# juliohm/GeoStatsSolvers.jl

Hardware: AMD Instinct MI355X
Metric: kriged domain points/sec (OK, 1000 3-D data, Matern-3/2, global neighbourhood) (higher is better)
Workload: dtype f64; 1 GPU; configs[1]: OK, 1000 3-D data -> 1000000 domain points per GPU, Matern-3/2 range 30, global neighbourhood; step = device fit + predict; points_per_gpu=1000000, ndata=1000, factor=replicated

## Files before the change

geostatssolvers.jl_amd/csrc/cokrig.hip:

```cpp
#include "krig_handle.h"
#include "mfma_f64.h"

#include <cmath>
#include <cstring>
#include <vector>

namespace gss {

template <int DIM>
__global__ __launch_bounds__(256) void cokrig_system_kernel(VgDev vg, const double* __restrict__ xd,
                                                            const int* __restrict__ var,
                                                            const double* __restrict__ tab, int n,
                                                            double* __restrict__ M, int64_t ldw) {
  const int j = blockIdx.x * 256 + threadIdx.x;
  const int i0 = blockIdx.y * 64;
  const int i1 = i0 + 64 < n ? i0 + 64 : n;
  if (j >= n) return;
  double c[DIM];
#pragma unroll
  for (int k = 0; k < DIM; ++k) c[k] = xd[(int64_t)j * DIM + k];
  const int vj = var[j];
  for (int i = i0; i < i1; ++i) {
    double x[DIM];
#pragma unroll
// ... 263 lines not shown
  for (int a = 0; a < nz; ++a) {
    h->c00[a] = tab[CO_C0 + a * CO_MAXZ + a];
    h->means[a] = tab[CO_MEANS + a];
  }
  std::memset(&h->ds, 0, sizeof(h->ds));
  h->ds.variant = variant;
  h->ds.dim = dim;
  for (int k = 0; k < 3; ++k) h->ds.inv_scale[k] = 1.0;
  h->nc = variant == GSS_KRIG_ORDINARY ? nz : 0;
  h->ds.nc = h->nc;
  h->N1 = n + h->nc;
  h->N1pad = round_up(h->N1 + 1, BK);
  h->ldw = round_up(h->N1 + 1, BM);

  hipStream_t s = to_stream(stream);
  GSS_TRY(h->z.alloc(sizeof(double) * (size_t)n));
  GSS_TRY(h->covar.alloc(sizeof(int32_t) * (size_t)n));
  GSS_TRY(h->cotab.alloc(sizeof(tab)));
  GSS_TRY(krig_upload_samples(h->fr, xdata, n, dim, &h->xdata, &h->xraw, s));
  GSS_HIP(hipMemcpyAsync(h->z.p, z, sizeof(double) * n, hipMemcpyHostToDevice, s));
  GSS_HIP(hipMemcpyAsync(h->covar.p, var, sizeof(int32_t) * n, hipMemcpyHostToDevice, s));
  GSS_HIP(hipMemcpyAsync(h->cotab.p, tab, sizeof(tab), hipMemcpyHostToDevice, s));
  {
    std::vector<double> xg((size_t)(n * dim)), zr((size_t)n);
    std::vector<int32_t> row((size_t)n);
    int64_t at[CO_MAXZ];
    h->co_off[0] = 0;
    for (int a = 0; a < CO_MAXZ; ++a) {
      at[a] = h->co_off[a];
      h->co_off[a + 1] = h->co_off[a] + per[a];
    }
    for (int64_t i = 0; i < n; ++i) {
      const int64_t j = at[var[i]]++;
      for (int k = 0; k < dim; ++k) xg[(size_t)(j * dim + k)] = xdata[i * dim + k];
      zr[(size_t)j] = z[i] - tab[CO_MEANS + var[i]];
      row[(size_t)j] = (int32_t)i;
    }
    GSS_TRY(h->co_zres.alloc(sizeof(double) * (size_t)n));
    GSS_TRY(h->co_row.alloc(sizeof(int32_t) * (size_t)n));
    GSS_TRY(krig_upload_samples(h->fr, xg.data(), n, dim, &h->co_xg, &h->co_xg_raw, s));
    GSS_HIP(hipMemcpyAsync(h->co_zres.p, zr.data(), sizeof(double) * n, hipMemcpyHostToDevice, s));
    GSS_HIP(hipMemcpyAsync(h->co_row.p, row.data(), sizeof(int32_t) * n, hipMemcpyHostToDevice, s));
    GSS_HIP(hipStreamSynchronize(s));
  }
  if (factor) {
    const bool async = (flags & GSS_KRIG_ASYNC_FIT) != 0;
    GSS_TRY(krig_factorize(h, s, async));
    if (!async) GSS_TRY(krig_fit_wait(h));
  }
  guard.h = nullptr;
  *out = h;
  return GSS_OK;
}

extern "C" {

int32_t gss_cokrig_create(gss_krig_t** out, const gss_variogram_t* structure, int32_t nz, const double* b0,
                          const double* b1, int32_t variant, const double* means, const double* xdata,
                          const double* z, const int32_t* var, int64_t n, int32_t flags, void* stream) {
  GSS_ENTRY();
  return cokrig_create_impl("gss_cokrig_create", true, out, structure, nz, b0, b1, variant, means, xdata, z, var, n,
                            flags, stream);
}

int32_t gss_cokrig_create_local(gss_krig_t** out, const gss_variogram_t* structure, int32_t nz, const double* b0,
                                const double* b1, int32_t variant, const double* means, const double* xdata,
                                const double* z, const int32_t* var, int64_t n, void* stream) {
  GSS_ENTRY();
  return cokrig_create_impl("gss_cokrig_create_local", false, out, structure, nz, b0, b1, variant, means, xdata, z, var,
                            n, 0, stream);
}

int32_t gss_cokrig_predict_global(gss_krig_t* h, const double* xdom, int64_t m, double* mean, double* variance,
                                  uint8_t* status, int32_t mem, void* stream) {
  GSS_ENTRY();
  GSS_REQUIRE(h != nullptr, "NULL handle");
  GSS_REQUIRE(h->nz > 0, "gss_cokrig_predict_global: the handle is not a cokriging system (gss_cokrig_create makes one)");
  GSS_REQUIRE(h->factored, "handle has no factor");
  GSS_REQUIRE(m >= 0 && (m == 0 || (xdom && mean && variance)), "gss_cokrig_predict_global: NULL array");
  if (m == 0) return GSS_OK;
  hipStream_t s = to_stream(stream);
  const int dim = h->dim, nz = h->nz;
  GSS_TRY(krig_quadform_attrs());

  int64_t mc = cokrig_chunk_cap(krig_chunk_points(h->N1pad * nz, m));
  DomainCall dc;
  Staged& sx = *dc.in(xdom, sizeof(double) * dim);
  Staged& smean = *dc.out(mean, sizeof(double), nz);
  Staged& svar = *dc.out(variance, sizeof(double), nz);
  Staged& sstat = *dc.out(status, 1, nz);
  GSS_TRY(dc.begin(mem, m, s, true, &h->fr));
  if (dc.piped && mc > HostPipe::PIECE) mc = HostPipe::PIECE;
  double *Rws = nullptr, *mpart = nullptr;
  GSS_TRY(krig_workspace(h->N1pad * nz, mc, s, &Rws, &mpart));
  const int64_t ldr = mc, blk = h->N1pad * ldr;
  const int seg_len = (int)((h->n + NSEG - 1) / NSEG);

  for (int64_t off = 0; off < m; off += mc) {
    const int64_t mv = (m - off) < mc ? (m - off) : mc;
    const int64_t cols = round_up(mv, 256);
    const double* x0 = sx.as<double>() + off * dim;
    GSS_TRY(dc.pipe.fetch(off, mv, s));
    const int nblk = (int)(cols / 256);
    const int nrows = (int)(h->N1pad - h->n);
    {
      ProfScope ps("cokrig_rhs", s);
      const double* xd = h->xdata.as<double>();
      const int* cv = h->covar.as<int>();
      const double* tab = h->cotab.as<double>();
      switch (dim) {
        case 1: GSS_TRY(launch_cokrig_rhs<1>(s, h->vg, xd, cv, tab, nz, (int)h->n, x0, mv, Rws, ldr, blk, seg_len, nblk)); break;
        case 2: GSS_TRY(launch_cokrig_rhs<2>(s, h->vg, xd, cv, tab, nz, (int)h->n, x0, mv, Rws, ldr, blk, seg_len, nblk)); break;
        default: GSS_TRY(launch_cokrig_rhs<3>(s, h->vg, xd, cv, tab, nz, (int)h->n, x0, mv, Rws, ldr, blk, seg_len, nblk)); break;
      }
      hipLaunchKernelGGL(cokrig_tail_rows_kernel, dim3((unsigned)(cols / 256)), dim3(256), 0, s, Rws, ldr, blk,
                         (int)h->n, h->nc, nrows, nz, cols);
      GSS_HIP(hipGetLastError());
    }
    GSS_TRY(krig_join_device(h, s));
    {
      ProfScope pq("krig_quadform", s);
      for (int t = 0; t < nz; ++t) {
        uint8_t* stp = status ? sstat.as<uint8_t>() + t * m + off : nullptr;
        launch_krig_quadform(h, Rws + t * blk, ldr, h->c00[t], h->means[t], mv, cols,
                             smean.as<double>() + t * m + off, svar.as<double>() + t * m + off, stp, mpart, s);
      }
    }
    GSS_HIP(hipGetLastError());
    GSS_TRY(dc.pipe.deliver(off, mv, s));
  }
  GSS_TRY(dc.finish(s));
  return krig_fit_wait(h);
}

int32_t gss_cokrig_predict_knn(gss_krig_t* h, const double* xdom, int64_t m, const int32_t* k, int32_t minneighbors,
                               double radius, const double* inv_radii, int32_t metric, double metric_param,
                               double* mean, double* variance, uint8_t* status, int32_t* idx_out, int32_t* count_out,
                               int32_t mem, void* stream) {
  GSS_ENTRY();
  GSS_REQUIRE(h != nullptr, "NULL handle");
  GSS_REQUIRE(h->nz > 0, "gss_cokrig_predict_knn: the handle is not a cokriging system (gss_cokrig_create and "
              "gss_cokrig_create_local make one)");
  const int nz = h->nz, dim = h->dim;
  int ksum = 0;
  GSS_TRY(cokrig_knn_counts(h, "gss_cokrig_predict_knn", "; gss_cokrig_predict_global uses every sample", k, &ksum));
  GSS_REQUIRE(m >= 0 && (m == 0 || (xdom && mean && variance)), "gss_cokrig_predict_knn: NULL array");

  hipStream_t s = to_stream(stream);
  CoGrouped g;
  cokrig_grouped(h, &g);
  Searcher sr[COL_MAXZ];
  GSS_TRY(cokrig_searchers(h, g, sr, metric, metric_param, radius, inv_radii, s));
  if (m == 0) return GSS_OK;
  DomainCall dc;
  dc.in(xdom, sizeof(double) * dim);
  Staged& smean = *dc.out(mean, sizeof(double), nz);
  Staged& svar = *dc.out(variance, sizeof(double), nz);
  Staged& sstat = *dc.out(status, 1, nz);
  Staged& sidx = *dc.out(idx_out, sizeof(int32_t) * (size_t)ksum);
  Staged& scnt = *dc.out(count_out, sizeof(int32_t) * (size_t)nz);
  GSS_TRY(dc.begin(mem, m, s, !sr[0].two_frames, &h->fr));
  GSS_TRY(cokrig_local_dev(h->vg, h->variant, dim, g, sr, k, minneighbors, dc.x(), sr[0].two_frames ? dc.x_raw : nullptr,
                           m, smean.as<double>(), svar.as<double>(), sstat.as<uint8_t>(), m, sidx.as<int>(),
                           scnt.as<int>(), s, &dc.pipe));
  return dc.finish(s);
}
// ... 3 lines not shown
```

geostatssolvers.jl_amd/csrc/krig.hip:

```cpp
#include "krig_handle.h"

#include "mfma_f64.h"

#include <mutex>

#include <cmath>
#include <cstdlib>
#include <cstring>
#include <type_traits>
#include <vector>

namespace gss {

template <int DIM>
__global__ __launch_bounds__(256) void drift_rows_kernel(DriftSpec ds, const double* __restrict__ x,
                                                         const double* __restrict__ drift_vals, int64_t npts,
                                                         int64_t ncols_pad, double* __restrict__ out, int64_t ld,
                                                         int nrows) {
  const int64_t p = (int64_t)blockIdx.x * 256 + threadIdx.x;
  if (p >= ncols_pad) return;
  const int64_t pc = p < npts ? p : npts - 1;
  double xs[DIM];
#pragma unroll
  for (int k = 0; k < DIM; ++k) xs[k] = (x[pc * DIM + k] - ds.center[k]) * ds.inv_scale[k];
// ... 468 lines not shown
    if (v > 0) ws = (size_t)v << 20;
  }
  int64_t cap = (int64_t)(ws / (sizeof(double) * (size_t)N1pad));
  const int64_t round = 512 * 128;
  cap = cap >= round ? cap / round * round : cap / 256 * 256;
  if (cap < 256) cap = 256;
  return round_up(m, 256) < cap ? round_up(m, 256) : cap;
}

struct KrigWorkspace {
  DevBuf R, mean_part;
  int64_t doubles = 0, mc = 0, nI = 0;
};
static KrigWorkspace g_ws;

int32_t gss::krig_workspace(int64_t N1pad, int64_t mc, hipStream_t s, double** R, double** mean_part) {
  const int64_t nI = (N1pad + BM - 1) / BM + 1;
  if (g_ws.doubles < N1pad * mc || g_ws.mc < mc || g_ws.nI < nI) {
    GSS_HIP(hipStreamSynchronize(s));
    g_ws.R.release();
    g_ws.mean_part.release();
    GSS_TRY(g_ws.R.alloc(sizeof(double) * (size_t)(N1pad * mc)));
    GSS_TRY(g_ws.mean_part.alloc(sizeof(double) * (size_t)((NSEG + 1 + nI) * mc)));
    g_ws.doubles = N1pad * mc;
    g_ws.mc = mc;
    g_ws.nI = nI;
  }
  *R = g_ws.R.as<double>();
  *mean_part = g_ws.mean_part.as<double>();
  return GSS_OK;
}

static int32_t launch_drift_rows(const gss_krig* h, const double* x, const double* drift_vals, int64_t npts,
                                 int64_t ncols_pad, double* out, int64_t ld, int nrows, hipStream_t s) {
  dim3 grid((unsigned)((ncols_pad + 255) / 256));
  switch (h->dim) {
    case 1:
      hipLaunchKernelGGL((drift_rows_kernel<1>), grid, dim3(256), 0, s, h->ds, x, drift_vals, npts, ncols_pad, out,
                         ld, nrows);
      break;
    case 2:
      hipLaunchKernelGGL((drift_rows_kernel<2>), grid, dim3(256), 0, s, h->ds, x, drift_vals, npts, ncols_pad, out,
                         ld, nrows);
      break;
    default:
      hipLaunchKernelGGL((drift_rows_kernel<3>), grid, dim3(256), 0, s, h->ds, x, drift_vals, npts, ncols_pad, out,
                         ld, nrows);
      break;
  }
  GSS_HIP(hipGetLastError());
  return GSS_OK;
}

__global__ void small_gram_kernel(const double* __restrict__ Bm, int nc, int64_t n, double* __restrict__ S, int lds) {
  const int c = blockIdx.x, c2 = blockIdx.y;
  if (c2 > c) return;
  double acc = 0.0;
  for (int64_t i = threadIdx.x; i < n; i += 64) acc = fma(Bm[(int64_t)c * n + i], Bm[(int64_t)c2 * n + i], acc);
#pragma unroll
  for (int off = 32; off >= 1; off >>= 1) acc += __shfl_xor(acc, off);
  if (threadIdx.x == 0) {
    S[c + c2 * lds] = acc;
    S[c2 + c * lds] = acc;
  }
}

__global__ void constraint_rows_kernel(const double* __restrict__ WS, int64_t ldws, const double* __restrict__ T,
                                       int nc, int64_t n, double* __restrict__ Wp_rows, int64_t ldw) {
  const int64_t j = (int64_t)blockIdx.x * 256 + threadIdx.x;
  if (j >= n) return;
  for (int i = 0; i < nc; ++i) {
    double acc = 0.0;
    for (int c = 0; c <= i; ++c) acc = fma(WS[i + c * ldws], T[(int64_t)c * n + j], acc);
    Wp_rows[i + j * ldw] = -acc;
  }
}

__global__ __launch_bounds__(256) void wd_row_kernel(const double* __restrict__ wd, int64_t N1,
                                                     double* __restrict__ row, int64_t ldw) {
  const int64_t k = (int64_t)blockIdx.x * 256 + threadIdx.x;
  if (k < N1) row[k * ldw] = wd[k];
}

struct FitPlan {
  double *M, *T, *Dinv, *Fd, *Bm, *S, *SDinv, *gwork, *zz, *u;
  int *info, *info2;
  int64_t szM, szS;
};

static int32_t krig_fit_plan(gss_krig* h, FitPlan* fp) {
  const int64_t n = h->n, N1pad = h->N1pad, ldw = h->ldw;
  const int64_t szM = ldw * N1pad;
  int64_t szT = n * n > (int64_t)MAX_NC * n ? n * n : (int64_t)MAX_NC * n;
  if (potrf_inverse_work_doubles(n) > szT) szT = potrf_inverse_work_doubles(n);
  const int64_t szDinv = 64 * 64;
  const int64_t szFd = (int64_t)MAX_NC * n, szBm = (int64_t)MAX_NC * n;
  const int64_t szS = 2 * MAX_NC * MAX_NC + 64 * 64;
  int64_t szGemv = gemv_work_doubles(false, ldw, ldw);
  if (gemv_work_doubles(true, ldw, ldw) > szGemv) szGemv = gemv_work_doubles(true, ldw, ldw);
  const int64_t szVec = 2 * ldw;
  DevBuf& ws = h->fit_ws;
  GSS_TRY(ws.alloc(sizeof(double) * (size_t)(szM + szT + szDinv + szFd + szBm + szS + szGemv + szVec) + 64));
  fp->M = ws.as<double>();
  fp->T = fp->M + szM;
  fp->Dinv = fp->T + szT;
  fp->Fd = fp->Dinv + szDinv;
  fp->Bm = fp->Fd + szFd;
  fp->S = fp->Bm + szBm;
  fp->SDinv = fp->S + MAX_NC * MAX_NC;
  fp->gwork = fp->S + szS;
  fp->zz = fp->gwork + szGemv;
  fp->u = fp->zz + ldw;
  fp->info = reinterpret_cast<int*>(fp->u + ldw);
  fp->info2 = fp->info + 1;
  fp->szM = szM;
  fp->szS = szS;
  return GSS_OK;
}

static int32_t krig_fit_enqueue(gss_krig* h, const FitPlan& fp, hipStream_t s) {
  const int64_t n = h->n, N1 = h->N1, ldw = h->ldw;
  const int nc = h->nc;
  double *M = fp.M, *T = fp.T, *Fd = fp.Fd, *Bm = fp.Bm, *S = fp.S, *SDinv = fp.SDinv;
  double *gwork = fp.gwork, *zz = fp.zz, *u = fp.u;
  int *info = fp.info, *info2 = fp.info2;
  const int64_t szM = fp.szM, szS = fp.szS;
  GSS_TRY(dev_zero_bytes(M, sizeof(double) * (size_t)szM, s));
  GSS_TRY(dev_zero_bytes(h->factor.p, h->factor.bytes, s));
  GSS_TRY(dev_zero_bytes(info2, sizeof(int), s));
  if (h->nz > 0) {
    GSS_TRY(cokrig_fit_system(h, M, s));
  } else {
    GSS_TRY(cov_pairwise_dev(h->vg, h->xdata.as<double>(), n, h->xdata.as<double>(), n, M, ldw, s));
  }
  double* Wp = h->Wp();
  GSS_TRY(potrf_inverse_f64(M, n, ldw, Wp, ldw, T, info, false, s, true));

  if (nc > 0) {
    GSS_TRY(dev_zero_bytes(S, sizeof(double) * (size_t)szS, s));
    if (h->nz > 0) {
      GSS_TRY(cokrig_fit_indicators(h, Fd, s));
    } else {
      GSS_TRY(launch_drift_rows(h, h->xdata.as<double>(), h->drift_data.as<double>(), n, n, Fd, n, nc, s));
    }
    for (int c = 0; c < nc; ++c) GSS_TRY(gemv_f64(false, n, n, Wp, ldw, Fd + (int64_t)c * n, Bm + (int64_t)c * n, gwork, s));
    hipLaunchKernelGGL(small_gram_kernel, dim3(nc, nc), dim3(64), 0, s, Bm, nc, n, S, MAX_NC);
    GSS_HIP(hipGetLastError());
    GSS_TRY(potrf_inverse_f64(S, nc, MAX_NC, Wp + n + n * ldw, ldw, SDinv, info2, false, s));
    for (int c = 0; c < nc; ++c) GSS_TRY(gemv_f64(true, n, n, Wp, ldw, Bm + (int64_t)c * n, T + (int64_t)c * n, gwork, s));
    hipLaunchKernelGGL(constraint_rows_kernel, dim3((unsigned)((n + 255) / 256)), dim3(256), 0, s, Wp + n + n * ldw, ldw, T,
                       nc, n, Wp + n, ldw);
    GSS_HIP(hipGetLastError());
  }

  GSS_TRY(dev_zero_bytes(zz, sizeof(double) * (size_t)(2 * ldw), s));
  GSS_TRY(dev_copy_f64(zz, h->z.as<double>(), n, s));
  if (h->nz > 0) {
    if (h->variant == GSS_KRIG_SIMPLE) cokrig_fit_center(h, zz, s);
  } else if (h->variant == GSS_KRIG_SIMPLE && h->sk_mean != 0.0) {
    hipLaunchKernelGGL(sub_scalar_kernel, dim3((unsigned)((n + 255) / 256)), dim3(256), 0, s, zz, n, h->sk_mean);
  }
  GSS_TRY(gemv_f64(false, N1, N1, Wp, ldw, zz, u, gwork, s));
  if (nc > 0) hipLaunchKernelGGL(flip_tail_kernel, dim3(1), dim3(256), 0, s, u, n, N1);
  GSS_TRY(gemv_f64(true, N1, N1, Wp, ldw, u, h->wd(), gwork, s));
  hipLaunchKernelGGL(wd_row_kernel, dim3((unsigned)((N1 + 255) / 256)), dim3(256), 0, s, h->wd(), N1, Wp + N1, ldw);
  GSS_HIP(hipGetLastError());
  return GSS_OK;
}

static hipStream_t krig_fit_stream() { return helper_stream(HELPER_FIT); }

static int32_t krig_factor_alloc(gss_krig* h) {
  if (h->factor.p) return GSS_OK;
  return h->factor.alloc(sizeof(double) * (size_t)(h->ldw * h->N1pad + h->N1pad));
}

int32_t gss::krig_factorize(gss_krig* h, hipStream_t s, bool async) {
  GSS_TRY(krig_factor_alloc(h));
  hipStream_t fs = s;
  if (async) {
    fs = krig_fit_stream();
    if (!fs) {
      async = false;
      fs = s;
    }
  }
  if (async) {
    ScopedEvent e0;
    GSS_HIP(e0.create());
    GSS_HIP(hipEventRecord(e0, s));
    GSS_HIP(hipStreamWaitEvent(fs, e0, 0));
    if (!h->fit_info_host) GSS_HIP(hipHostMalloc(reinterpret_cast<void**>(&h->fit_info_host), 2 * sizeof(int), hipHostMallocDefault));
  }
  FitPlan fp;
  GSS_TRY(krig_fit_plan(h, &fp));
  GSS_TRY(krig_fit_enqueue(h, fp, fs));
  h->fit_info = fp.info;
  h->fit_stream = fs;
  h->fit_async = async;
  if (async) GSS_HIP(hipMemcpyAsync(h->fit_info_host, fp.info, 2 * sizeof(int), hipMemcpyDeviceToHost, fs));
  if (!h->fit_done) GSS_HIP(hipEventCreateWithFlags(&h->fit_done, hipEventDisableTiming));
  GSS_HIP(hipEventRecord(h->fit_done, fs));
  h->fit_pending = true;
  h->factored = true;
  return GSS_OK;
}

int32_t gss::krig_join_device(gss_krig* h, hipStream_t s) {
  if (h->fit_pending && h->fit_done && h->fit_stream != s) GSS_HIP(hipStreamWaitEvent(s, h->fit_done, 0));
  return GSS_OK;
}

int32_t gss::krig_fit_wait(gss_krig* h) {
  if (!h->fit_pending) return GSS_OK;
  h->fit_pending = false;
  GSS_HIP(hipEventSynchronize(h->fit_done));
  int hinfo[2] = {0, 0};
  if (h->fit_async) {
    hinfo[0] = h->fit_info_host[0];
    hinfo[1] = h->fit_info_host[1];
  } else {
    GSS_HIP(hipMemcpy(hinfo, h->fit_info, 2 * sizeof(int), hipMemcpyDeviceToHost));
  }
  h->fit_ws.release();
  h->fit_info = nullptr;
  if (hinfo[0] < 0) {
    h->factored = false;
    static thread_local bool retrying = false;
    if (!retrying) {
      potrf_panel_disable();
      retrying = true;
      int32_t rc = krig_factorize(h, h->fit_stream, false);
      if (rc == GSS_OK) rc = krig_fit_wait(h);
      retrying = false;
      return rc;
    }
    set_error("kriging fit: the factorisation kernel gave up waiting at a grid barrier");
    return GSS_ERR_HIP;
  }
  if (hinfo[0] != 0) {
    h->factored = false;
    set_error("kriging covariance matrix is not positive definite (pivot %d of %lld); add a nugget or remove "
              "duplicate samples", hinfo[0] - 1, (long long)h->n);
    return GSS_ERR_NOT_POSDEF;
  }
  if (hinfo[1] != 0) {
    h->factored = false;
    set_error("drift functions are linearly dependent on the sample locations (constraint %d)", hinfo[1] - 1);
    return GSS_ERR_NOT_POSDEF;
  }
  return GSS_OK;
}

void gss::launch_krig_quadform(const gss_krig* h, const double* Rws, int64_t ldr, double c00, double mean0,
                                 int64_t mv, int64_t cols, double* mean_out, double* var_out, uint8_t* stp,
                                 double* qpart, hipStream_t s) {
  const int nstrips = (int)(cols / BN);
  const int nI = (int)((h->N1 + BM) / BM);
#define GSS_K3_ARGS(S0, NS) h->Wp(), h->ldw, (int)h->N1pad, (int)h->n, (int)h->N1, Rws, ldr, c00, mean0, mv, \
                            mean_out, var_out, stp, qpart, (S0), (NS)
  const int nmain = (nstrips / 512) * 512;
  const int nrem = nstrips - nmain;
  if (nmain > 0)
    hipLaunchKernelGGL((krig_quadform_kernel<false>), dim3((unsigned)nmain), dim3(256), QUADFORM_LDS_BYTES, s,
                       GSS_K3_ARGS(0, nmain));
  if (nrem > 0) {
    const unsigned grid = (unsigned)(8 * ((nrem + 7) / 8) * nI);
    hipLaunchKernelGGL((krig_quadform_kernel<true>), dim3(grid), dim3(256), QUADFORM_LDS_BYTES, s,
                       GSS_K3_ARGS(nmain, nrem));
    const int64_t pbeg = (int64_t)nmain * BN;
    if (mv > pbeg)
      hipLaunchKernelGGL(krig_finish_kernel, dim3((unsigned)((mv - pbeg + 255) / 256)), dim3(256), 0, s, qpart + pbeg,
                         nI, ldr, c00, mv - pbeg, var_out + pbeg, stp ? stp + pbeg : nullptr);
  }
#undef GSS_K3_ARGS
}

int32_t gss::krig_quadform_attrs() {
  static uint64_t attr_set = 0;
  if (first_on_this_device(attr_set)) {
    GSS_HIP(hipFuncSetAttribute(reinterpret_cast<const void*>(krig_quadform_kernel<false>),
                                hipFuncAttributeMaxDynamicSharedMemorySize, (int)QUADFORM_LDS_BYTES));
    GSS_HIP(hipFuncSetAttribute(reinterpret_cast<const void*>(krig_quadform_kernel<true>),
                                hipFuncAttributeMaxDynamicSharedMemorySize, (int)QUADFORM_LDS_BYTES));
  }
  return GSS_OK;
}

int32_t gss::krig_upload_samples(const Frame& fr, const double* xhost, int64_t n, int dim, DevBuf* x, DevBuf* xraw,
                                 hipStream_t s) {
  const size_t bytes = sizeof(double) * (size_t)(n * dim);
  GSS_TRY(x->alloc(bytes));
  if (!fr.on) {
    GSS_HIP(hipMemcpyAsync(x->p, xhost, bytes, hipMemcpyHostToDevice, s));
    return GSS_OK;
  }
  GSS_TRY(xraw->alloc(bytes));
  GSS_HIP(hipMemcpyAsync(xraw->p, xhost, bytes, hipMemcpyHostToDevice, s));
  return frame_apply_dev(fr, xraw->as<double>(), n, x->as<double>(), s);
// ... 66 lines not shown
      break;
    }
    case GSS_KRIG_EXTDRIFT:
      GSS_REQUIRE(ndrift >= 1 && ndrift <= MAX_NC && drift_data != nullptr, "external drift needs 1..%d drifts",
                  MAX_NC);
      h->nc = ndrift;
      break;
    default:
      GSS_REQUIRE(false, "unknown kriging variant %d", variant);
  }
  h->ds.nc = h->nc;
  if ((flags & GSS_KRIG_NO_FACTOR) == 0)
    GSS_REQUIRE(n + h->nc >= 1 && n >= h->nc, "fewer samples (%lld) than drift constraints (%d)", (long long)n,
                h->nc);
  h->N1 = n + h->nc;
  h->N1pad = round_up(h->N1 + 1, BK);
  h->ldw = round_up(h->N1 + 1, BM);

  hipStream_t s = to_stream(stream);
  GSS_TRY(h->z.alloc(sizeof(double) * (size_t)n));
  GSS_TRY(krig_upload_samples(h->fr, xdata, n, h->dim, &h->xdata, &h->xraw, s));
  GSS_HIP(hipMemcpyAsync(h->z.p, z, sizeof(double) * n, hipMemcpyHostToDevice, s));
  if (variant == GSS_KRIG_EXTDRIFT) {
    GSS_TRY(h->drift_data.alloc(sizeof(double) * (size_t)(n * ndrift)));
    GSS_HIP(hipMemcpyAsync(h->drift_data.p, drift_data, sizeof(double) * n * ndrift, hipMemcpyHostToDevice, s));
  }
  GSS_HIP(hipStreamSynchronize(s));
  if ((flags & GSS_KRIG_NO_FACTOR) == 0) {
    const bool async = (flags & GSS_KRIG_ASYNC_FIT) != 0;
    GSS_TRY(krig_factorize(h, s, async));
    if (!async) GSS_TRY(krig_fit_wait(h));
  }
  guard.h = nullptr;
  *out = h;
  return GSS_OK;
}

int32_t gss_krig_destroy(gss_krig_t* h) {
  GSS_ENTRY();
  delete h;
  return GSS_OK;
}

int32_t gss_krig_info(const gss_krig_t* h, int64_t* n, int32_t* nc) {
  GSS_ENTRY();
  GSS_REQUIRE(h != nullptr, "NULL handle");
  if (n) *n = h->n;
  if (nc) *nc = h->nc;
  return GSS_OK;
}

int32_t gss_krig_factor_buffer(gss_krig_t* h, void** dev_ptr, int64_t* bytes) {
  GSS_ENTRY();
  GSS_REQUIRE(h != nullptr && dev_ptr != nullptr && bytes != nullptr, "NULL argument");
  GSS_TRY(krig_fit_wait(h));
  GSS_TRY(krig_factor_alloc(h));
  *dev_ptr = h->factor.p;
  *bytes = (int64_t)(sizeof(double) * (size_t)(h->ldw * h->N1pad + h->N1pad));
  return GSS_OK;
}

int32_t gss_krig_adopt_factor(gss_krig_t* h) {
  GSS_ENTRY();
  GSS_REQUIRE(h != nullptr, "NULL handle");
  GSS_REQUIRE(h->factor.p != nullptr, "gss_krig_adopt_factor: no factor has arrived (gss_krig_factor_buffer hands out "
                                      "the buffer to fill)");
  h->factored = true;
  return GSS_OK;
}

int32_t gss_krig_predict_global(gss_krig_t* h, const double* xdom, const double* drift_dom, int64_t m,
                                double* mean, double* var, uint8_t* status, int32_t mem, void* stream) {
  GSS_ENTRY();
  GSS_REQUIRE(h != nullptr, "NULL handle");
  GSS_TRY(krig_refuse_cokrig(h, "gss_krig_predict_global"));
  GSS_REQUIRE(h->factored, "handle has no factor (created with GSS_KRIG_NO_FACTOR and never adopted one)");
  GSS_REQUIRE(m >= 0 && (m == 0 || (xdom && mean && var)), "gss_krig_predict_global: NULL array");
  GSS_REQUIRE(h->variant != GSS_KRIG_EXTDRIFT || drift_dom != nullptr, "external drift values missing");
  if (m == 0) return GSS_OK;
  hipStream_t s = to_stream(stream);
  const int dim = h->dim;

  GSS_TRY(krig_quadform_attrs());

  int64_t mc = krig_chunk_points(h->N1pad, m);
  DomainCall dc;
  Staged& sx = *dc.in(xdom, sizeof(double) * dim);
  Staged& sd = *dc.in(h->variant == GSS_KRIG_EXTDRIFT ? drift_dom : nullptr, sizeof(double) * h->ndrift);
  Staged& smean = *dc.out(mean, sizeof(double));
  Staged& svar = *dc.out(var, sizeof(double));
  Staged& sstat = *dc.out(status, 1);
  GSS_TRY(dc.begin(mem, m, s, true, &h->fr));
  if (dc.piped && mc > HostPipe::PIECE) mc = HostPipe::PIECE;
  double *Rws = nullptr, *mpart = nullptr;
  GSS_TRY(krig_workspace(h->N1pad, mc, s, &Rws, &mpart));
  const int64_t ldr = mc;
  const int seg_len = (int)((h->n + NSEG - 1) / NSEG);

  for (int64_t off = 0; off < m; off += mc) {
    const int64_t mv = (m - off) < mc ? (m - off) : mc;
    const int64_t cols = round_up(mv, 256);
    const double* x0 = sx.as<double>() + off * dim;
    GSS_TRY(dc.pipe.fetch(off, mv, s));
    const int nblk = (int)(cols / 256);
    const int nrows = (int)(h->N1pad - h->n);
    {
      ProfScope ps("krig_rhs", s);
      if (h->block_nsub > 0) {
        const dim3 gb((unsigned)((ldr + 255) / 256));
        const double* bc = h->block_cell;
        switch (dim) {
          case 1: hipLaunchKernelGGL(krig_rhs_block_kernel<1>, gb, dim3(256), 0, s, h->vg, h->xdata.as<double>(), (int)h->n, x0, mv, Rws, ldr, h->block_nsub, bc[0], bc[1], bc[2]); break;
          case 2: hipLaunchKernelGGL(krig_rhs_block_kernel<2>, gb, dim3(256), 0, s, h->vg, h->xdata.as<double>(), (int)h->n, x0, mv, Rws, ldr, h->block_nsub, bc[0], bc[1], bc[2]); break;
          default: hipLaunchKernelGGL(krig_rhs_block_kernel<3>, gb, dim3(256), 0, s, h->vg, h->xdata.as<double>(), (int)h->n, x0, mv, Rws, ldr, h->block_nsub, bc[0], bc[1], bc[2]); break;
        }
      } else
      switch (dim) {
        case 1: GSS_TRY(launch_krig_rhs<1>(s, h->vg, h->xdata.as<double>(), (int)h->n, x0, mv, Rws, ldr, seg_len, nblk)); break;
        case 2: GSS_TRY(launch_krig_rhs<2>(s, h->vg, h->xdata.as<double>(), (int)h->n, x0, mv, Rws, ldr, seg_len, nblk)); break;
        default: GSS_TRY(launch_krig_rhs<3>(s, h->vg, h->xdata.as<double>(), (int)h->n, x0, mv, Rws, ldr, seg_len, nblk)); break;
      }
    GSS_HIP(hipGetLastError());
    if (nrows > 0) {
      const double* dv = h->variant == GSS_KRIG_EXTDRIFT ? sd.as<double>() + off * h->ndrift : nullptr;
      GSS_TRY(launch_drift_rows(h, x0, dv, mv, cols, Rws + h->n * ldr, ldr, nrows, s));
    }
    }
    GSS_TRY(krig_join_device(h, s));
    ProfScope pq("krig_quadform", s);
    {
      const double mean0 = h->variant == GSS_KRIG_SIMPLE ? h->sk_mean : 0.0;
      uint8_t* stp = status ? sstat.as<uint8_t>() + off : nullptr;
      const double c00 = h->block_nsub > 0 ? h->block_cvv : h->vg.sill;
      launch_krig_quadform(h, Rws, ldr, c00, mean0, mv, cols, smean.as<double>() + off, svar.as<double>() + off, stp,
                           mpart, s);
    }
    GSS_HIP(hipGetLastError());
    GSS_TRY(dc.pipe.deliver(off, mv, s));
  }
  GSS_TRY(dc.finish(s));
  return krig_fit_wait(h);
}

int32_t gss_krig_set_block_support(gss_krig_t* h, const double* cell, int32_t nsub, void* stream) {
  GSS_ENTRY();
  GSS_REQUIRE(h != nullptr, "NULL handle");
  GSS_TRY(krig_refuse_cokrig(h, "gss_krig_set_block_support"));
  if (nsub <= 0 || cell == nullptr) {
    h->block_nsub = 0;
    return GSS_OK;
  }
  GSS_REQUIRE(nsub <= 8, "block support: at most 8 samples per axis (got %d)", nsub);
  GSS_REQUIRE(nsub == 0 || cell == nullptr || !h->fr.on,
              "block support with a rotated variogram is not available (its sub-cell offsets are axis-aligned in "
              "the raw frame, DESIGN.md section 7)");
  GSS_REQUIRE(h->vg.kind != GSS_VG_POWER, "block support needs a stationary variogram");
  GSS_REQUIRE(h->variant != GSS_KRIG_EXTDRIFT && !(h->variant == GSS_KRIG_UNIVERSAL && h->degree > 1),
              "block support: simple / ordinary kriging or a drift of degree <= 1 (the cell average of a linear drift is "
              "its value at the centroid; higher degrees and external drifts would need their own cell averages)");
  for (int a = 0; a < h->dim; ++a) GSS_REQUIRE(cell[a] > 0.0, "block support: cell sizes must be positive");
  hipStream_t s = to_stream(stream);
  DevBuf out;
  GSS_TRY(out.alloc(sizeof(double)));
  double c[3] = {0.0, 0.0, 0.0};
  for (int a = 0; a < h->dim; ++a) c[a] = cell[a];
  switch (h->dim) {
// ... 116 lines not shown
```

geostatssolvers.jl_amd/csrc/krig_handle.h:

```cpp
#pragma once

#include "gss_internal.h"
#include "cokrig.h"

namespace gss {

constexpr int MAX_NC = 64;
constexpr int NSEG = 4;

struct DriftSpec {
  int variant;
  int nc;
  int dim;
  signed char e[MAX_NC][3];
  double center[3];
  double inv_scale[3];
};

}

struct gss_krig {
  gss::VgDev vg;
  int variant = GSS_KRIG_ORDINARY;
  double sk_mean = 0.0;
  int degree = 0;
  int ndrift = 0;
  int dim = 0;
  int64_t n = 0;
  int nc = 0;
  int64_t N1 = 0, N1pad = 0, ldw = 0;
  gss::DriftSpec ds;
  gss::DevBuf xdata, z, drift_data;
  gss::Frame fr;
  gss::DevBuf xraw;
  gss::DevBuf factor;
  gss::DevBuf fit_ws;
  hipEvent_t fit_done = nullptr;
  bool fit_pending = false;
  int* fit_info = nullptr;
  hipStream_t fit_stream = nullptr;
  bool fit_async = false;
  int* fit_info_host = nullptr;
  ~gss_krig() {
    if (fit_pending && fit_done) (void)hipEventSynchronize(fit_done);
    if (fit_done) (void)hipEventDestroy(fit_done);
    if (fit_info_host) (void)hipHostFree(fit_info_host);
  }
  bool factored = false;
  int block_nsub = 0;
  double block_cell[3] = {0.0, 0.0, 0.0};
  double block_cvv = 0.0;
  int nz = 0;
  gss::DevBuf covar, cotab;
  double c00[gss::CO_MAXZ] = {}, means[gss::CO_MAXZ] = {};
  gss::DevBuf co_xg, co_xg_raw, co_zres, co_row;
  int64_t co_off[gss::CO_MAXZ + 1] = {};
  double* Wp() const { return factor.as<double>(); }
  double* wd() const { return factor.as<double>() + ldw * N1pad; }
};

namespace gss {
int32_t krig_local_dev(const VgDev& vg, int variant, int nc, int dim, const signed char* exps, double inv_scale,
                       double sk_mean, Searcher& sr, const double* xdata, const double* z, const double* drift_data,
                       const double* x0, const double* x0_raw, const double* drift_dom, int64_t m, int k,
                       int minneighbors, double* mean, double* var, uint8_t* status, int* idx_out, int* count_out,
                       hipStream_t s, HostPipe* pipe, int block_nsub, const double* block_cell, double block_cvv,
                       const KnnMask* mask = nullptr);

int64_t krig_chunk_points(int64_t N1pad, int64_t m);
int32_t krig_workspace(int64_t N1pad, int64_t mc, hipStream_t s, double** R, double** mean_part);
int32_t krig_upload_samples(const Frame& fr, const double* xhost, int64_t n, int dim, DevBuf* x, DevBuf* xraw,
                            hipStream_t s);
int32_t krig_factorize(gss_krig* h, hipStream_t s, bool async = false);
int32_t krig_join_device(gss_krig* h, hipStream_t s);
int32_t krig_fit_wait(gss_krig* h);
void launch_krig_quadform(const gss_krig* h, const double* Rws, int64_t ldr, double c00, double mean0, int64_t mv,
                          int64_t cols, double* mean_out, double* var_out, uint8_t* stp, double* qpart, hipStream_t s);
int32_t krig_quadform_attrs();
int32_t krig_refuse_cokrig(const gss_krig* h, const char* who);

int32_t cokrig_fit_system(const gss_krig* h, double* M, hipStream_t s);
int32_t cokrig_fit_indicators(const gss_krig* h, double* Fd, hipStream_t s);
void cokrig_fit_center(const gss_krig* h, double* zz, hipStream_t s);
void cokrig_grouped(const gss_krig* h, CoGrouped* g);
int32_t cokrig_knn_counts(const gss_krig* h, const char* who, const char* clamp_note, const int32_t* k, int* ksum);
int32_t cokrig_searchers(const gss_krig* h, const CoGrouped& g, Searcher* sr, int32_t metric, double metric_param,
                         double radius, const double* inv_radii, hipStream_t s);

}
```

Before: 52.85 million points/s.

## Fuse constraint-tail fit into custom kernels and overlap predict with tail via event

For small drift counts, the post-factorization fit tail (per-column gemvs, small Cholesky, constraint rows, weight vector) is replaced by a few custom kernels: chunked partial mat-vecs, a single-block kernel that does the constraint Gram, its Cholesky and inverse, and a closing kernel. A new event is recorded right after the main inverse so the predict stream can start covariance assembly while the fit tail still runs. The goal is to cut launch count and serial tail latency in the fit and hide the rest behind prediction. It adds partial-sum workspace and relies on the predict's later join to order reads of the final weights.

```diff
diff --git a/geostatssolvers.jl_amd/csrc/cokrig.hip b/geostatssolvers.jl_amd/csrc/cokrig.hip
--- a/geostatssolvers.jl_amd/csrc/cokrig.hip
+++ b/geostatssolvers.jl_amd/csrc/cokrig.hip
@@ -369,6 +369,7 @@
   hipStream_t s = to_stream(stream);
   const int dim = h->dim, nz = h->nz;
   GSS_TRY(krig_quadform_attrs());
+  GSS_TRY(krig_order_assembly(h, s));
 
   int64_t mc = cokrig_chunk_cap(krig_chunk_points(h->N1pad * nz, m));
   DomainCall dc;
diff --git a/geostatssolvers.jl_amd/csrc/krig.hip b/geostatssolvers.jl_amd/csrc/krig.hip
--- a/geostatssolvers.jl_amd/csrc/krig.hip
+++ b/geostatssolvers.jl_amd/csrc/krig.hip
@@ -574,17 +574,192 @@
   if (k < N1) row[k * ldw] = wd[k];
 }
 
+constexpr int TAIL_MAX_NC = 16;
+constexpr int TAIL_NV = TAIL_MAX_NC + 1;
+constexpr int TAIL_CHUNK = 64;
+constexpr int TAIL_TCHUNK = 256;
+
+__global__ __launch_bounds__(64) void fit_mv_n_partial_kernel(int64_t n, const double* __restrict__ W, int64_t ldw,
+                                                              const double* __restrict__ X, int nv,
+                                                              double* __restrict__ partial) {
+  const int64_t i = (int64_t)blockIdx.x * 64 + threadIdx.x;
+  const int64_t j0 = (int64_t)blockIdx.y * TAIL_CHUNK;
+  const int64_t j1 = j0 + TAIL_CHUNK < n ? j0 + TAIL_CHUNK : n;
+  if (i >= n) return;
+  double acc[TAIL_NV];
+#pragma unroll
+  for (int v = 0; v < TAIL_NV; ++v) acc[v] = 0.0;
+  for (int64_t j = j0; j < j1; ++j) {
+    const double a = W[i + j * ldw];
+#pragma unroll
+    for (int v = 0; v < TAIL_NV; ++v)
+      if (v < nv) acc[v] = fma(a, X[(int64_t)v * n + j], acc[v]);
+  }
+#pragma unroll
+  for (int v = 0; v < TAIL_NV; ++v)
+    if (v < nv) partial[((int64_t)blockIdx.y * nv + v) * n + i] = acc[v];
+}
+
+__global__ __launch_bounds__(64) void fit_mv_t_partial_kernel(int64_t n, const double* __restrict__ W, int64_t ldw,
+                                                              const double* __restrict__ Y, int nyp, int nv,
+                                                              double* __restrict__ partial) {
+  const int64_t j = blockIdx.x;
+  const int64_t i0 = (int64_t)blockIdx.y * TAIL_TCHUNK;
+  const int64_t i1 = i0 + TAIL_TCHUNK < n ? i0 + TAIL_TCHUNK : n;
+  const int lane = threadIdx.x;
+  double acc[TAIL_NV];
+#pragma unroll
+  for (int v = 0; v < TAIL_NV; ++v) acc[v] = 0.0;
+  for (int64_t i = i0 + lane; i < i1; i += 64) {
+    const double a = W[i + j * ldw];
+#pragma unroll
+    for (int v = 0; v < TAIL_NV; ++v)
+      if (v < nv) {
+        double y = 0.0;
+        for (int q = 0; q < nyp; ++q) y += Y[((int64_t)q * nv + v) * n + i];
+        acc[v] = fma(a, y, acc[v]);
+      }
+  }
+#pragma unroll
+  for (int v = 0; v < TAIL_NV; ++v)
+    if (v < nv) {
+      double r = acc[v];
+#pragma unroll
+      for (int off = 32; off >= 1; off >>= 1) r += __shfl_xor(r, off);
+      if (lane == 0) partial[((int64_t)blockIdx.y * nv + v) * n + j] = r;
+    }
+}
+
+__global__ __launch_bounds__(1024) void fit_constraint_block_kernel(const double* __restrict__ partial, int np,
+                                                                    int64_t n, int nc, double* Y,
+                                                                    double* __restrict__ Wss, int64_t ldw,
+                                                                    double* __restrict__ sm, int* __restrict__ info2) {
+  __shared__ double S[TAIL_NV][TAIL_NV];
+  __shared__ double WS[TAIL_MAX_NC][TAIL_NV];
+  __shared__ double d0[TAIL_MAX_NC], ub[TAIL_MAX_NC], g[TAIL_MAX_NC];
+  const int tid = threadIdx.x, lane = tid & 63, wave = tid >> 6;
+  const int nv = nc + 1;
+  for (int64_t e = tid; e < (int64_t)nv * n; e += 1024) {
+    const int64_t v = e / n, i = e - v * n;
+    double acc = 0.0;
+    for (int p = 0; p < np; ++p) acc += partial[((int64_t)p * nv + v) * n + i];
+    Y[e] = acc;
+  }
+  if (tid < TAIL_MAX_NC * TAIL_NV) (&WS[0][0])[tid] = 0.0;
+  __syncthreads();
+  int e = 0;
+  for (int c = 0; c <= nc; ++c)
+    for (int c2 = 0; c2 <= c && c2 < nc; ++c2, ++e) {
+      if ((e & 15) != wave) continue;
+      double acc = 0.0;
+      for (int64_t i = lane; i < n; i += 64) acc = fma(Y[(int64_t)c * n + i], Y[(int64_t)c2 * n + i], acc);
+#pragma unroll
+      for (int off = 32; off >= 1; off >>= 1) acc += __shfl_xor(acc, off);
+      if (lane == 0) S[c][c2] = acc;
+    }
+  __syncthreads();
+  if (tid < nc) d0[tid] = S[tid][tid];
+  __syncthreads();
+  const int i = tid & 15, j = tid >> 4;
+  const bool el = tid < 256 && i < nc && j < nc;
+  int bad = 0;
+  for (int k = 0; k < nc; ++k) {
+    double p = S[k][k];
+    __syncthreads();
+    if (!(p > 4.0 * nc * 2.220446049250313e-16 * d0[k])) {
+      if (bad == 0) bad = k + 1;
+      p = 1.0;
+    }
+    const double r = sqrt(p);
+    if (el && j == k && i >= k) S[i][k] = (i == k) ? r : S[i][k] / r;
+    __syncthreads();
+    if (el && j > k && i >= j) S[i][j] = fma(-S[i][k], S[j][k], S[i][j]);
+    __syncthreads();
+  }
+  if (tid < nc) {
+    const int c = tid;
+    WS[c][c] = 1.0 / S[c][c];
+    for (int r = c + 1; r < nc; ++r) {
+      double acc = 0.0;
+      for (int k = c; k < r; ++k) acc = fma(S[r][k], WS[k][c], acc);
+      WS[r][c] = -acc / S[r][r];
+    }
+  }
+  __syncthreads();
+  if (tid < nc) {
+    double acc = 0.0;
+    for (int c = 0; c <= tid; ++c) acc = fma(WS[tid][c], S[nc][c], acc);
+    ub[tid] = -acc;
+  }
+  __syncthreads();
+  if (tid < nc) {
+    double acc = 0.0;
+    for (int r = tid; r < nc; ++r) acc = fma(WS[r][tid], ub[r], acc);
+    g[tid] = acc;
+  }
+  __syncthreads();
+  if (tid < 256) {
+    sm[i + TAIL_MAX_NC * j] = WS[i][j];
+    if (el && j <= i) Wss[i + (int64_t)j * ldw] = WS[i][j];
+  }
+  if (tid < TAIL_MAX_NC) sm[TAIL_MAX_NC * TAIL_MAX_NC + tid] = tid < nc ? g[tid] : 0.0;
+  if (tid == 0 && bad != 0) *info2 = bad;
+}
+
+__global__ __launch_bounds__(256) void fit_close_kernel(const double* __restrict__ partial, int np, int64_t n, int nc,
+                                                        const double* __restrict__ sm, double* __restrict__ Wp,
+                                                        int64_t ldw, double* __restrict__ wd) {
+  const int64_t k = (int64_t)blockIdx.x * 256 + threadIdx.x;
+  const int64_t N1 = n + nc;
+  const int nv = nc + 1;
+  if (k >= N1) return;
+  double w;
+  if (k < n) {
+    double t[TAIL_MAX_NC];
+#pragma unroll
+    for (int c = 0; c < TAIL_MAX_NC; ++c) {
+      double acc = 0.0;
+      if (c < nc)
+        for (int p = 0; p < np; ++p) acc += partial[((int64_t)p * nv + c) * n + k];
+      t[c] = acc;
+    }
+    w = 0.0;
+    for (int p = 0; p < np; ++p) w += partial[((int64_t)p * nv + nc) * n + k];
+#pragma unroll
+    for (int i = 0; i < TAIL_MAX_NC; ++i)
+      if (i < nc) {
+        double acc = 0.0;
+#pragma unroll
+        for (int c = 0; c <= i; ++c) acc = fma(sm[i + TAIL_MAX_NC * c], t[c], acc);
+        Wp[n + i + k * ldw] = -acc;
+      }
+#pragma unroll
+    for (int c = 0; c < TAIL_MAX_NC; ++c)
+      if (c < nc) w = fma(t[c], sm[TAIL_MAX_NC * TAIL_MAX_NC + c], w);
+  } else {
+    w = -sm[TAIL_MAX_NC * TAIL_MAX_NC + (k - n)];
+  }
+  wd[k] = w;
+  Wp[N1 + k * ldw] = w;
+}
+
 struct FitPlan {
-  double *M, *T, *Dinv, *Fd, *Bm, *S, *SDinv, *gwork, *zz, *u;
+  double *M, *T, *Dinv, *Fd, *Bm, *S, *SDinv, *gwork, *zz, *u, *P2;
   int *info, *info2;
   int64_t szM, szS;
 };
+
+static bool fit_short_tail(const gss_krig* h) { return h->nc <= TAIL_MAX_NC; }
 
 static int32_t krig_fit_plan(gss_krig* h, FitPlan* fp) {
   const int64_t n = h->n, N1pad = h->N1pad, ldw = h->ldw;
   const int64_t szM = ldw * N1pad;
   int64_t szT = n * n > (int64_t)MAX_NC * n ? n * n : (int64_t)MAX_NC * n;
   if (potrf_inverse_work_doubles(n) > szT) szT = potrf_inverse_work_doubles(n);
+  const int64_t nv = h->nc + 1;
+  const int64_t szP1 = fit_short_tail(h) ? (n + TAIL_CHUNK - 1) / TAIL_CHUNK * nv * n : 0;
+  const int64_t szP2 = fit_short_tail(h) ? (n + TAIL_TCHUNK - 1) / TAIL_TCHUNK * nv * n : 0;
+  if (szP1 > szT) szT = szP1;
   const int64_t szDinv = 64 * 64;
   const int64_t szFd = (int64_t)MAX_NC * n, szBm = (int64_t)MAX_NC * n;
   const int64_t szS = 2 * MAX_NC * MAX_NC + 64 * 64;
@@ -592,7 +767,7 @@
   if (gemv_work_doubles(true, ldw, ldw) > szGemv) szGemv = gemv_work_doubles(true, ldw, ldw);
   const int64_t szVec = 2 * ldw;
   DevBuf& ws = h->fit_ws;
-  GSS_TRY(ws.alloc(sizeof(double) * (size_t)(szM + szT + szDinv + szFd + szBm + szS + szGemv + szVec) + 64));
+  GSS_TRY(ws.alloc(sizeof(double) * (size_t)(szM + szT + szDinv + szFd + szBm + szS + szGemv + szVec + szP2) + 64));
   fp->M = ws.as<double>();
   fp->T = fp->M + szM;
   fp->Dinv = fp->T + szT;
@@ -603,20 +778,22 @@
   fp->gwork = fp->S + szS;
   fp->zz = fp->gwork + szGemv;
   fp->u = fp->zz + ldw;
-  fp->info = reinterpret_cast<int*>(fp->u + ldw);
+  fp->P2 = fp->u + ldw;
+  fp->info = reinterpret_cast<int*>(fp->P2 + szP2);
   fp->info2 = fp->info + 1;
   fp->szM = szM;
   fp->szS = szS;
   return GSS_OK;
 }
 
-static int32_t krig_fit_enqueue(gss_krig* h, const FitPlan& fp, hipStream_t s) {
+static int32_t krig_fit_enqueue(gss_krig* h, const FitPlan& fp, hipStream_t s, hipEvent_t factored) {
   const int64_t n = h->n, N1 = h->N1, ldw = h->ldw;
   const int nc = h->nc;
   double *M = fp.M, *T = fp.T, *Fd = fp.Fd, *Bm = fp.Bm, *S = fp.S, *SDinv = fp.SDinv;
   double *gwork = fp.gwork, *zz = fp.zz, *u = fp.u;
   int *info = fp.info, *info2 = fp.info2;
   const int64_t szM = fp.szM, szS = fp.szS;
+  const bool tail = fit_short_tail(h);
   GSS_TRY(dev_zero_bytes(M, sizeof(double) * (size_t)szM, s));
   GSS_TRY(dev_zero_bytes(h->factor.p, h->factor.bytes, s));
   GSS_TRY(dev_zero_bytes(info2, sizeof(int), s));
@@ -625,35 +802,59 @@
   } else {
     GSS_TRY(cov_pairwise_dev(h->vg, h->xdata.as<double>(), n, h->xdata.as<double>(), n, M, ldw, s));
   }
-  double* Wp = h->Wp();
-  GSS_TRY(potrf_inverse_f64(M, n, ldw, Wp, ldw, T, info, false, s, true));
-
+  double* zc = tail ? Fd + (int64_t)nc * n : zz;
   if (nc > 0) {
-    GSS_TRY(dev_zero_bytes(S, sizeof(double) * (size_t)szS, s));
     if (h->nz > 0) {
       GSS_TRY(cokrig_fit_indicators(h, Fd, s));
     } else {
       GSS_TRY(launch_drift_rows(h, h->xdata.as<double>(), h->drift_data.as<double>(), n, n, Fd, n, nc, s));
     }
-    for (int c = 0; c < nc; ++c) GSS_TRY(gemv_f64(false, n, n, Wp, ldw, Fd + (int64_t)c * n, Bm + (int64_t)c * n, gwork, s));
-    hipLaunchKernelGGL(small_gram_kernel, dim3(nc, nc), dim3(64), 0, s, Bm, nc, n, S, MAX_NC);
+  }
+  if (!tail) GSS_TRY(dev_zero_bytes(zz, sizeof(double) * (size_t)(2 * ldw), s));
+  GSS_TRY(dev_copy_f64(zc, h->z.as<double>(), n, s));
+  if (h->nz > 0) {
+    if (h->variant == GSS_KRIG_SIMPLE) cokrig_fit_center(h, zc, s);
+  } else if (h->variant == GSS_KRIG_SIMPLE && h->sk_mean != 0.0) {
+    hipLaunchKernelGGL(sub_scalar_kernel, dim3((unsigned)((n + 255) / 256)), dim3(256), 0, s, zc, n, h->sk_mean);
+  }
+  GSS_HIP(hipGetLastError());
+  double* Wp = h->Wp();
+  GSS_TRY(potrf_inverse_f64(M, n, ldw, Wp, ldw, T, info, false, s, true));
+  if (factored) GSS_HIP(hipEventRecord(factored, s));
+
+  if (tail) {
+    const int nv = nc + 1;
+    const int np1 = (int)((n + TAIL_CHUNK - 1) / TAIL_CHUNK), np2 = (int)((n + TAIL_TCHUNK - 1) / TAIL_TCHUNK);
+    double *P1 = T, *P2 = fp.P2, *sm = S;
+    hipLaunchKernelGGL(fit_mv_n_partial_kernel, dim3((unsigned)((n + 63) / 64), (unsigned)np1), dim3(64), 0, s, n, Wp, ldw,
+                       Fd, nv, P1);
+    if (nc > 0) {
+      hipLaunchKernelGGL(fit_constraint_block_kernel, dim3(1), dim3(1024), 0, s, P1, np1, n, nc, Bm, Wp + n + n * ldw,
+                         ldw, sm, info2);
+      hipLaunchKernelGGL(fit_mv_t_partial_kernel, dim3((unsigned)n, (unsigned)np2), dim3(64), 0, s, n, Wp, ldw, Bm, 1, nv,
+                         P2);
+    } else {
+      hipLaunchKernelGGL(fit_mv_t_partial_kernel, dim3((unsigned)n, (unsigned)np2), dim3(64), 0, s, n, Wp, ldw, P1, np1,
+                         nv, P2);
+    }
+    hipLaunchKernelGGL(fit_close_kernel, dim3((unsigned)((N1 + 255) / 256)), dim3(256), 0, s, P2, np2, n, nc, sm, Wp, ldw,
+                       h->wd());
     GSS_HIP(hipGetLastError());
-    GSS_TRY(potrf_inverse_f64(S, nc, MAX_NC, Wp + n + n * ldw, ldw, SDinv, info2, false, s));
-    for (int c = 0; c < nc; ++c) GSS_TRY(gemv_f64(true, n, n, Wp, ldw, Bm + (int64_t)c * n, T + (int64_t)c * n, gwork, s));
-    hipLaunchKernelGGL(constraint_rows_kernel, dim3((unsigned)((n + 255) / 256)), dim3(256), 0, s, Wp + n + n * ldw, ldw, T,
-                       nc, n, Wp + n, ldw);
-    GSS_HIP(hipGetLastError());
-  }
-
-  GSS_TRY(dev_zero_bytes(zz, sizeof(double) * (size_t)(2 * ldw), s));
-  GSS_TRY(dev_copy_f64(zz, h->z.as<double>(), n, s));
-  if (h->nz > 0) {
-    if (h->variant == GSS_KRIG_SIMPLE) cokrig_fit_center(h, zz, s);
-  } else if (h->variant == GSS_KRIG_SIMPLE && h->sk_mean != 0.0) {
-    hipLaunchKernelGGL(sub_scalar_kernel, dim3((unsigned)((n + 255) / 256)), dim3(256), 0, s, zz, n, h->sk_mean);
-  }
+    return GSS_OK;
+  }
+
+  GSS_TRY(dev_zero_bytes(S, sizeof(double) * (size_t)szS, s));
+  for (int c = 0; c < nc; ++c) GSS_TRY(gemv_f64(false, n, n, Wp, ldw, Fd + (int64_t)c * n, Bm + (int64_t)c * n, gwork, s));
+  hipLaunchKernelGGL(small_gram_kernel, dim3(nc, nc), dim3(64), 0, s, Bm, nc, n, S, MAX_NC);
+  GSS_HIP(hipGetLastError());
+  GSS_TRY(potrf_inverse_f64(S, nc, MAX_NC, Wp + n + n * ldw, ldw, SDinv, info2, false, s));
+  for (int c = 0; c < nc; ++c) GSS_TRY(gemv_f64(true, n, n, Wp, ldw, Bm + (int64_t)c * n, T + (int64_t)c * n, gwork, s));
+  hipLaunchKernelGGL(constraint_rows_kernel, dim3((unsigned)((n + 255) / 256)), dim3(256), 0, s, Wp + n + n * ldw, ldw, T,
+                     nc, n, Wp + n, ldw);
+  GSS_HIP(hipGetLastError());
+
   GSS_TRY(gemv_f64(false, N1, N1, Wp, ldw, zz, u, gwork, s));
-  if (nc > 0) hipLaunchKernelGGL(flip_tail_kernel, dim3(1), dim3(256), 0, s, u, n, N1);
+  hipLaunchKernelGGL(flip_tail_kernel, dim3(1), dim3(256), 0, s, u, n, N1);
   GSS_TRY(gemv_f64(true, N1, N1, Wp, ldw, u, h->wd(), gwork, s));
   hipLaunchKernelGGL(wd_row_kernel, dim3((unsigned)((N1 + 255) / 256)), dim3(256), 0, s, h->wd(), N1, Wp + N1, ldw);
   GSS_HIP(hipGetLastError());
@@ -683,10 +884,11 @@
     GSS_HIP(hipEventRecord(e0, s));
     GSS_HIP(hipStreamWaitEvent(fs, e0, 0));
     if (!h->fit_info_host) GSS_HIP(hipHostMalloc(reinterpret_cast<void**>(&h->fit_info_host), 2 * sizeof(int), hipHostMallocDefault));
+    if (!h->fit_factored) GSS_HIP(hipEventCreateWithFlags(&h->fit_factored, hipEventDisableTiming));
   }
   FitPlan fp;
   GSS_TRY(krig_fit_plan(h, &fp));
-  GSS_TRY(krig_fit_enqueue(h, fp, fs));
+  GSS_TRY(krig_fit_enqueue(h, fp, fs, async ? h->fit_factored : nullptr));
   h->fit_info = fp.info;
   h->fit_stream = fs;
   h->fit_async = async;
@@ -703,10 +905,28 @@
   return GSS_OK;
 }
 
+static bool krig_join_at_assembly() {
+  static const bool v = [] {
+    const char* e = std::getenv("GSS_KRIG_FIT_JOIN");
+    return e != nullptr && std::strcmp(e, "assembly") == 0;
+  }();
+  return v;
+}
+
+int32_t gss::krig_order_assembly(gss_krig* h, hipStream_t s) {
+  if (!h->fit_pending || !h->fit_factored || h->fit_stream == s) return GSS_OK;
+  GSS_HIP(hipStreamWaitEvent(s, krig_join_at_assembly() ? h->fit_done : h->fit_factored, 0));
+  return GSS_OK;
+}
+
 int32_t gss::krig_fit_wait(gss_krig* h) {
   if (!h->fit_pending) return GSS_OK;
   h->fit_pending = false;
   GSS_HIP(hipEventSynchronize(h->fit_done));
+  if (h->fit_factored) {
+    (void)hipEventDestroy(h->fit_factored);
+    h->fit_factored = nullptr;
+  }
   int hinfo[2] = {0, 0};
   if (h->fit_async) {
     hinfo[0] = h->fit_info_host[0];
@@ -939,6 +1159,7 @@
   const int dim = h->dim;
 
   GSS_TRY(krig_quadform_attrs());
+  GSS_TRY(krig_order_assembly(h, s));
 
   int64_t mc = krig_chunk_points(h->N1pad, m);
   DomainCall dc;
diff --git a/geostatssolvers.jl_amd/csrc/krig_handle.h b/geostatssolvers.jl_amd/csrc/krig_handle.h
--- a/geostatssolvers.jl_amd/csrc/krig_handle.h
+++ b/geostatssolvers.jl_amd/csrc/krig_handle.h
@@ -41,9 +41,11 @@
   hipStream_t fit_stream = nullptr;
   bool fit_async = false;
   int* fit_info_host = nullptr;
+  hipEvent_t fit_factored = nullptr;
   ~gss_krig() {
     if (fit_pending && fit_done) (void)hipEventSynchronize(fit_done);
     if (fit_done) (void)hipEventDestroy(fit_done);
+    if (fit_factored) (void)hipEventDestroy(fit_factored);
     if (fit_info_host) (void)hipHostFree(fit_info_host);
   }
   bool factored = false;
@@ -73,6 +75,7 @@
                             hipStream_t s);
 int32_t krig_factorize(gss_krig* h, hipStream_t s, bool async = false);
 int32_t krig_join_device(gss_krig* h, hipStream_t s);
+int32_t krig_order_assembly(gss_krig* h, hipStream_t s);
 int32_t krig_fit_wait(gss_krig* h);
 void launch_krig_quadform(const gss_krig* h, const double* Rws, int64_t ldr, double c00, double mean0, int64_t mv,
                           int64_t cols, double* mean_out, double* var_out, uint8_t* stp, double* qpart, hipStream_t s);
```

Result: no change. 52.63 million points/s (-0.4%).
